# baumgach/PHiSeg-code

Hardware: AMD Instinct MI355X
Metric: training images/sec (ELBO step) phiseg_7_5 128x128 LIDC (higher is better)
Workload: dtype bf16; 1 GPU; phiseg_7_5 LIDC 128x128x1, 2 classes, bf16, batch norm, batch 64 per GPU, full ELBO training step (fwd + CE + KL + bwd + Adam); global_batch=64, parallelism=dp1

## Files before the change

### include/phx_debug.h

```cpp
#ifndef PHX_DEBUG_H
#define PHX_DEBUG_H
#ifdef __cplusplus
extern "C" {
#endif
int phx_debug_conv_policy(int large_maps, int big_tiles);
int phx_debug_pair_kernel_grid(int blocks);
int phx_debug_layer_norm_policy(int one_launch_max, int chunk);
#ifdef __cplusplus
}
#endif
#endif
```

### phiseg_code_amd/csrc/conv_c32.hip

```cpp
#include <stdlib.h>

#include <type_traits>

#include "phx_common.h"

namespace {

constexpr int C32_AI = 39;
constexpr int C32_NPL = 10;
constexpr int C32_STAGE = 40 * 1024;
constexpr int C32_PROW = 34 * 64;
constexpr int C32_LDS = 2 * C32_STAGE;

typedef __attribute__((address_space(3))) void* lds_ptr_t;

__device__ __forceinline__ unsigned lds_offset(const void* p) {
    return (unsigned)(uintptr_t)(const __attribute__((address_space(3))) unsigned char*)p;
}

__device__ unsigned long long* g_c32_trace = nullptr;
#define C32_TRACE(slot)                                                                          \
    do {                                                                                         \
        if (g_c32_trace && blockIdx.x == 0 && threadIdx.x == 0 && (slot) < 512)                   \
            g_c32_trace[slot] = __builtin_readcyclecounter();                                     \
    } while (0)

template <bool BIASACT, bool XF = false>
__global__ __launch_bounds__(256, 2) void k_conv3x3_c32(const unsigned short* __restrict__ x, const unsigned short* __restrict__ wpk,
                                                        unsigned short* __restrict__ y, const float* __restrict__ bias, int act,
                                                        float* __restrict__ stats_partial, int B, int H, int W, int tiles_x,
                                                        int tiles_y, int ntiles, const float* __restrict__ oscale, int stats_nrep, unsigned mgx, unsigned mgy,
                                                        const float* __restrict__ xscale = nullptr, const float* __restrict__ xshift = nullptr) {
    extern __shared__ __attribute__((aligned(16))) unsigned char smem[];
    const int wave = threadIdx.x >> 6, lane = threadIdx.x & 63;
    const int l31 = lane & 31, khalf = lane >> 5;

    bf16x8 fb[9][2];
#pragma unroll
    for (int tap = 0; tap < 9; ++tap)
#pragma unroll
        for (int ks = 0; ks < 2; ++ks)
            fb[tap][ks] = *reinterpret_cast<const bf16x8*>(wpk + ((tap * 32 + l31) * 32 + (ks * 2 + khalf) * 8));

    unsigned rel[C32_NPL], edge[C32_NPL];
#pragma unroll
    for (int n = 0; n < C32_NPL; ++n) {
        const int j = wave + 4 * n;
        const int e = j * 64 + lane, pp = e >> 2, slot = e & 3;
        const int py = pp / 34, px = pp - py * 34;
// ... 194 lines not shown
            const float s1 = s1v[0] + s1v[1], s2 = s2v[0] + s2v[1];
            const float a = s1 + __shfl_xor(s1, 32, 64);
            const float bq = s2 + __shfl_xor(s2, 32, 64);
            if (khalf == 0) {
                red[(wave * 2 + 0) * 32 + l31] = a;
                red[(wave * 2 + 1) * 32 + l31] = bq;
            }
            asm volatile("s_waitcnt lgkmcnt(0)\n\ts_barrier" ::: "memory");
            if (threadIdx.x < 64) {
                const int which = threadIdx.x >> 5, n = threadIdx.x & 31;
                float r0, r1, r2, r3;
                asm volatile("ds_read_b32 %0, %4\n\tds_read_b32 %1, %4 offset:256\n\tds_read_b32 %2, %4 offset:512\n\t"
                             "ds_read_b32 %3, %4 offset:768\n\ts_waitcnt lgkmcnt(0)"
                             : "=&v"(r0), "=&v"(r1), "=&v"(r2), "=&v"(r3)
                             : "v"(lds_offset(red + which * 32 + n))
                             : "memory");
                const float v = (r0 + r1) + (r2 + r3);
                if (stats_nrep > 0) atomicAdd(&stats_partial[((size_t)(t % stats_nrep) * 32 + n) * 2 + which], v);
                else stats_partial[((size_t)t * 2 + which) * 32 + n] = v;
            }
        }
    }
}

}

int phx_c32_set_trace(void* dev_buf) {
    PHX_CHECK_HIP(hipMemcpyToSymbol(HIP_SYMBOL(g_c32_trace), &dev_buf, sizeof(void*)));
    return PHX_OK;
}
bool phx_c32_enabled() { return true; }

int phx_c32_launch(const void* x, const void* wpk, void* y, const float* bias, int act, float* stats_partial, int B, int H, int W,
                   const float* oscale, int stats_nrep, void* stream, const float* xscale, const float* xshift) {
    const int tiles_x = W / 32, tiles_y = H / 16, ntiles = B * tiles_x * tiles_y;
    const int cap = 512;
    const int grid = ntiles < cap ? ntiles : cap;
    const bool ba = bias != nullptr || act != PHX_ACT_ID || oscale != nullptr;
    PHX_REQUIRE(ntiles < 65536, PHX_E_SHAPE, "conv3x3_c32: more than 65535 tiles");
    const unsigned mgx = (unsigned)((0x100000000ull + tiles_x - 1) / tiles_x), mgy = (unsigned)((0x100000000ull + tiles_y - 1) / tiles_y);
    if (xscale != nullptr) {
        PHX_REQUIRE(xshift != nullptr && !ba, PHX_E_INVAL, "conv3x3_c32: the input transform takes a plain epilogue");
        PHX_CHECK_HIP(hipFuncSetAttribute((const void*)k_conv3x3_c32<false, true>, hipFuncAttributeMaxDynamicSharedMemorySize, 160 * 1024));
        hipLaunchKernelGGL((k_conv3x3_c32<false, true>), dim3(grid), dim3(256), C32_LDS, (hipStream_t)stream, (const unsigned short*)x,
                           (const unsigned short*)wpk, (unsigned short*)y, bias, act, stats_partial, B, H, W, tiles_x, tiles_y, ntiles,
                           oscale, stats_nrep, mgx, mgy, xscale, xshift);
    } else if (ba) {
        PHX_CHECK_HIP(hipFuncSetAttribute((const void*)k_conv3x3_c32<true>, hipFuncAttributeMaxDynamicSharedMemorySize, 160 * 1024));
        hipLaunchKernelGGL((k_conv3x3_c32<true>), dim3(grid), dim3(256), C32_LDS, (hipStream_t)stream, (const unsigned short*)x,
                           (const unsigned short*)wpk, (unsigned short*)y, bias, act, stats_partial, B, H, W, tiles_x, tiles_y, ntiles,
                           oscale, stats_nrep, mgx, mgy, (const float*)nullptr, (const float*)nullptr);
    } else {
        PHX_CHECK_HIP(hipFuncSetAttribute((const void*)k_conv3x3_c32<false>, hipFuncAttributeMaxDynamicSharedMemorySize, 160 * 1024));
        hipLaunchKernelGGL((k_conv3x3_c32<false>), dim3(grid), dim3(256), C32_LDS, (hipStream_t)stream, (const unsigned short*)x,
                           (const unsigned short*)wpk, (unsigned short*)y, bias, act, stats_partial, B, H, W, tiles_x, tiles_y, ntiles,
                           oscale, stats_nrep, mgx, mgy, (const float*)nullptr, (const float*)nullptr);
    }
    PHX_CHECK_LAUNCH();
    return PHX_OK;
}
// ... 1 lines not shown
```

### phiseg_code_amd/csrc/conv_common.h

```cpp
#pragma once
#include <stdlib.h>

#include <type_traits>

#include "phx_common.h"
#include <cstring>

#ifndef PHX_ABLATE
#define PHX_ABLATE 0
#endif
#ifndef PHX_FRAG_DEPTH
#define PHX_FRAG_DEPTH 2
#endif
#define KC 32
#define ROWB 80
#define PITCH16 1536

struct MTile {
    int tws, ths, tb, tiles_x, tiles_y, tiles_b;
    unsigned mpw, mpp;
    int rpitch, ipitch;
};
static void mtile_magic(MTile* g) {
    const unsigned pw = (1u << g->tws) + 2, ph = (1u << g->ths) + 2;
    g->mpw = ((1u << 20) + pw - 1) / pw;
    g->mpp = ((1u << 20) + pw * ph - 1) / (pw * ph);
    g->rpitch = (int)pw * ROWB;
    g->ipitch = (int)ph * g->rpitch;
    if (g->tws == 3 && g->ths == 3) { g->rpitch = 56 * 16; g->ipitch = 560 * 16; }
    else if (g->tws == 2 && g->ths == 2) { g->rpitch = 36 * 16; g->ipitch = 224 * 16; }
    else if (g->tws == 1 && g->ths == 1) { g->rpitch = 22 * 16; g->ipitch = 92 * 16; }
}
__device__ __forceinline__ void patch_coords(const MTile& g, int pp, int pw, int ph, int* px, int* py, int* pb) {
    const int b = (int)(__umul24((unsigned)pp, g.mpp) >> 20);
    const int rem = pp - (int)__umul24((unsigned)b, (unsigned)(pw * ph));
// ... 59 lines not shown
```

### phiseg_code_amd/csrc/conv_mfma.hip

```cpp
#include "conv_common.h"

#ifdef PHX_DEBUG_BUILD
static int g_ws_policy = 1;
static int g_tile_policy = 1;
#else
static constexpr int g_ws_policy = 1, g_tile_policy = 1;
#endif

static bool fwd_big_tiles(int B, int H, int W, int K, int N) {
    if (!g_tile_policy || H % 32 != 0 || W % 16 != 0) return false;
    if (g_tile_policy == 2) return true;
    return (N % 128 == 0 || (N == 32 && K >= 128)) && (long)B * (H / 32) * (W / 16) >= 512;
}
static bool fwd_ws64(int B, int H, int W, int K, int N) {
    if (!g_ws_policy || H % 16 != 0 || W % 32 != 0 || N % 32 != 0 || K % 32 != 0) return false;
    if ((long)B * (H / 16) * (W / 32) >= 65536 || (double)B * H * W * (K > N ? K : N) >= 2147483648.0) return false;
    if (g_ws_policy >= 2) return true;
    if (N % 64 != 0 && K > 64) return false;
    return (long)B * (H / 16) * (W / 32) * (N / (N % 64 == 0 ? 64 : 32)) >= 512;
}
static MTile make_mtile_fwd(int B, int H, int W, int K, int N, bool allow_dma = true) {
    if (allow_dma && fwd_ws64(B, H, W, K, N)) {
        MTile g;
        g.tws = 5; g.ths = 4; g.tb = 1;
// ... 98 lines not shown
}
struct UnpadJob {
    const float* dw_pad; float* dw;
    int Cin, Cin_pad, Cout, ntap, blk0, reserved;
};
static_assert(sizeof(UnpadJob) == 40, "phx_unpad_filter_grad_multi: 40-byte job records (include/phx.h)");
__global__ void k_unpad_rows_acc_multi(const UnpadJob* __restrict__ jobs, int njobs) {
    int lo = 0, hi = njobs - 1;
    while (lo < hi) {
        const int mid = (lo + hi + 1) >> 1;
        if (jobs[mid].blk0 <= (int)blockIdx.x) lo = mid; else hi = mid - 1;
    }
    const UnpadJob j = jobs[lo];
    const int nblk = (lo + 1 < njobs ? jobs[lo + 1].blk0 : (int)gridDim.x) - j.blk0;
    if ((int)blockIdx.x < j.blk0 || nblk < 1) return;
    const int n = j.ntap * j.Cin * j.Cout;
    for (int i = (blockIdx.x - j.blk0) * blockDim.x + threadIdx.x; i < n; i += nblk * blockDim.x) {
        const int co = i % j.Cout, ci = (i / j.Cout) % j.Cin, t = j.ntap == 1 ? 4 : i / (j.Cout * j.Cin);
        j.dw[i] += j.dw_pad[((size_t)t * j.Cin_pad + ci) * j.Cout + co];
    }
}

int phx_c32_set_trace(void* dev_buf);
int phx_wgrad_set_debug(void* trace_buf, void* blocklog_buf, int which);
bool phx_c32_enabled();
int phx_c32_launch(const void* x, const void* wpk, void* y, const float* bias, int act, float* stats_partial, int B, int H, int W,
                   const float* oscale, int stats_nrep, void* stream, const float* xscale = nullptr, const float* xshift = nullptr);
struct Dual;
bool phx_pp_shape_ok(int B, int H, int W, int K, int N);
int phx_pp_set_trace(void* dev_buf);
int phx_pp_set_grid(int blocks);
int phx_pp_launch(const void* x, const void* wpk, void* y, const float* bias, int act, float* stats_partial, int B, int H, int W,
                  int K, int N, const float* oscale, int stats_nrep, Dual du, int dbg, void* stream);

struct EpiOpts {
    int stats_atomic;
    const float* oscale;
    float* y_f32;
    bool keep_slices;
};

struct XForm {
    const float *gamma, *beta;
    float eps;
    int G, act;
    unsigned short* a_out;
// ... 737 lines not shown
    return PHX_OK;
}

int phx_debug_set_trace(void* dev_buf) {
    if (int rc = phx_c32_set_trace(dev_buf)) return rc;
    if (int rc = phx_pp_set_trace(dev_buf)) return rc;
    if (int rc = phx_wgrad_set_debug(dev_buf, nullptr, 0)) return rc;
    unsigned long long* p = (unsigned long long*)dev_buf;
    PHX_CHECK_HIP(hipMemcpyToSymbol(HIP_SYMBOL(g_phx_trace), &p, sizeof(p)));
    return PHX_OK;
}

#ifdef PHX_DEBUG_BUILD
int phx_debug_conv_policy(int large_maps, int big_tiles) {
    PHX_REQUIRE(large_maps >= 0 && large_maps <= 2 && big_tiles >= 0 && big_tiles <= 2, PHX_E_INVAL, "debug_conv_policy: 0 never, 1 policy, 2 force");
    g_ws_policy = large_maps;
    g_tile_policy = big_tiles;
    return PHX_OK;
}

int phx_debug_pair_kernel_grid(int blocks) {
    PHX_REQUIRE(blocks >= 0, PHX_E_INVAL, "debug_pair_kernel_grid: blocks >= 0 (0: one per CU)");
    return phx_pp_set_grid(blocks);
}
#endif

int phx_debug_set_blocklog(void* dev_buf) {
    if (int rc = phx_wgrad_set_debug(nullptr, dev_buf, 1)) return rc;
    unsigned long long* p = (unsigned long long*)dev_buf;
    PHX_CHECK_HIP(hipMemcpyToSymbol(HIP_SYMBOL(g_phx_blocklog), &p, sizeof(p)));
    return PHX_OK;
}

static int q_tiles(int B, int H, int W, int K, int N) {
    MTile g = make_mtile_fwd(B, H, W, K, N);
    return g.tiles_x * g.tiles_y * g.tiles_b;
}

static int q_tiles_dual(int B, int H, int W, int K, int N) {
    MTile g = fwd_ws64(B, H, W, K, N) ? make_mtile_fwd(B, H, W, K, N) : make_mtile(B, H, W);
    return g.tiles_x * g.tiles_y * g.tiles_b;
}

static int fwd_ksplit(int B, int H, int W, int K, int N) {
    if (fwd_big_tiles(B, H, W, K, N)) return 1;
    MTile g = make_mtile(B, H, W);
// ... 285 lines not shown
```

### phiseg_code_amd/csrc/conv_wgrad.hip

```cpp
#include "conv_common.h"

template <int RB>
__device__ __forceinline__ int wswz(int pix, int byte_in_row) {
    if (RB == 128) return pix * 128 + (byte_in_row ^ (((pix >> 1) & 1) << 6));
    return pix * RB + byte_in_row;
}

template <int TCI, int TCO, bool BIGP, bool FAST16>
__device__ __forceinline__ void conv3x3_wgrad_body(const unsigned short* __restrict__ x0, const unsigned short* __restrict__ dy,
                                                   float* __restrict__ dw, float* __restrict__ ws, int B, int H, int W, int Cin,
                                                   int Cout, MTile g, int ntiles, int tiles_per_block, const int bx,
                                                   const int by, const int bz, const int gdx, const int gdy,
                                                   const unsigned short* __restrict__ x2 = nullptr, const int K1 = 0) {
    const bool src2 = x2 != nullptr && by * TCI >= K1;
    const unsigned short* __restrict__ x = src2 ? x2 : x0;
    const int xC = x2 == nullptr ? Cin : (src2 ? Cin - K1 : K1);
    const int xc0 = by * TCI - (src2 ? K1 : 0);
    constexpr int WI = TCI / 32, WJ = TCO / 32, WK = 4 / (WI * WJ);
    constexpr int RBX = TCI * 2, RBD = TCO * 2;
    constexpr int QX = TCI / 8, QD = TCO / 8;
    constexpr int NXI = ((BIGP ? 1024 : 400) * QX + 255) / 256;
    const int tw = 1 << g.tws, th = 1 << g.ths;
    const int pw = tw + 2, ph = th + 2;
    const int npatch = g.tb * ph * pw;
// ... 81 lines not shown
        if constexpr (PHX_ABLATE & 16) return;
        if constexpr (idx < NXI) {
            const int gx = ptx0 + (planx[idx] & 255) - 1, gy = pty0 + ((planx[idx] >> 8) & 255) - 1, gb = pb0 + (planx[idx] >> 16);
            const bool ok = planx[idx] >= 0 && gx >= 0 && gx < W && gy >= 0 && gy < H && gb < B;
            const unsigned vo = ok ? (unsigned)(((gb * H + gy) * W + gx) * xC * 2 + qxb) : 0xffffffffu;
            rx[idx] = __builtin_amdgcn_raw_buffer_load_b128(rsx, vo, xc0 * 2, 0);
        } else if constexpr (idx < NXI + QD) {
            constexpr int it = idx - NXI;
            const int ox = ptx0 + (pland[it] & 255), oy = pty0 + ((pland[it] >> 8) & 255), ob = pb0 + (pland[it] >> 16);
            const bool ok = ox < W && oy < H && ob < B;
            const unsigned vo = ok ? (unsigned)(((ob * H + oy) * W + ox) * Cout * 2 + qdb) : 0xffffffffu;
            rd[it] = __builtin_amdgcn_raw_buffer_load_b128(rsd, vo, co0 * 2, 0);
        }
    };
    auto prefetch_range = [&](auto self, auto lo, auto hi) {
        constexpr int l = decltype(lo)::value, h = decltype(hi)::value;
        if constexpr (l < h && l < NXI + QD) {
            prefetch_piece(lo);
            self(self, std::integral_constant<int, l + 1>(), hi);
        }
    };
    const int t_begin = bx * tiles_per_block;
    const int t_end = min(ntiles, t_begin + tiles_per_block);
    PHX_BLOCKLOG_BEGIN();
    PHX_TRACE(0);
    if (t_begin < t_end) {
        if constexpr (FAST16) {
            decode(t_begin);
            prefetch_range(prefetch_range, std::integral_constant<int, 0>(), std::integral_constant<int, NXI + QD>());
        } else {
            prefetch(t_begin);
        }
    }
    PHX_TRACE(1);

    for (int t = t_begin; t < t_end; ++t) {
        __syncthreads();
        if (t == t_begin) PHX_TRACE(2);
#pragma unroll
        for (int it = 0; it < NXI; ++it) {
            const int i = threadIdx.x + it * 256;
            if (planx[it] >= 0) *reinterpret_cast<u32x4*>(sX + wswz<RBX>(i / QX, (i % QX) * 16)) = rx[it];
        }
#pragma unroll
        for (int it = 0; it < QD; ++it) {
            const int i = threadIdx.x + it * 256;
            *reinterpret_cast<u32x4*>(sD + wswz<RBD>(i / QD, (i % QD) * 16)) = rd[it];
        }
        __syncthreads();
        if (t == t_begin) PHX_TRACE(3);
        const bool more = t + 1 < t_end;
        if constexpr (FAST16) { if (more) decode(t + 1); }
        else if (more) prefetch(t + 1);
        if (t == t_begin) PHX_TRACE(4);
        if (FAST16) {
            constexpr int NSTEP = 16 / WK;
            s16x4 fd[2][2], fx[2][9][2];
            auto read_step = [&](unsigned xb, unsigned db, auto parc, auto bufc) {
                constexpr int P = decltype(parc)::value;
                constexpr int Bf = decltype(bufc)::value;
                fd[Bf][0] = __builtin_amdgcn_ds_read_tr16_b64_v4i16((s16x4 __attribute__((address_space(3)))*)(smem + db + dcon[0]));
                fd[Bf][1] = __builtin_amdgcn_ds_read_tr16_b64_v4i16((s16x4 __attribute__((address_space(3)))*)(smem + db + dcon[1]));
#pragma unroll
                for (int kh = 0; kh < 3; ++kh)
#pragma unroll
                    for (int kw = 0; kw < 3; ++kw) {
                        const int par = (P + kh) & 1;
                        fx[Bf][kh * 3 + kw][0] = __builtin_amdgcn_ds_read_tr16_b64_v4i16(
                            (s16x4 __attribute__((address_space(3)))*)(smem + xb + kh * 18 * RBX + xcon[0][kw][par]));
                        fx[Bf][kh * 3 + kw][1] = __builtin_amdgcn_ds_read_tr16_b64_v4i16(
                            (s16x4 __attribute__((address_space(3)))*)(smem + xb + kh * 18 * RBX + xcon[1][kw][par]));
                    }
            };
            auto mfma_step = [&](auto bufc) {
                constexpr int Bf = decltype(bufc)::value;
                const s16x8 dtmp = {fd[Bf][0][0], fd[Bf][0][1], fd[Bf][0][2], fd[Bf][0][3], fd[Bf][1][0], fd[Bf][1][1], fd[Bf][1][2], fd[Bf][1][3]};
                const bf16x8 bfrag = __builtin_bit_cast(bf16x8, dtmp);
// ... 46 lines not shown
                }
                const s16x4 d0 = __builtin_amdgcn_ds_read_tr16_b64_v4i16(
                    (s16x4 __attribute__((address_space(3)))*)(sD + wswz<RBD>(mpix[0], chan_byte_d)));
                const s16x4 d1 = __builtin_amdgcn_ds_read_tr16_b64_v4i16(
                    (s16x4 __attribute__((address_space(3)))*)(sD + wswz<RBD>(mpix[1], chan_byte_d)));
                const s16x8 dtmp = {d0[0], d0[1], d0[2], d0[3], d1[0], d1[1], d1[2], d1[3]};
                const bf16x8 bfrag = __builtin_bit_cast(bf16x8, dtmp);
    #pragma unroll
                for (int kh = 0; kh < 3; ++kh)
    #pragma unroll
                    for (int kw = 0; kw < 3; ++kw) {
                        const int sh = kh * pw + kw;
                        const s16x4 a0 = __builtin_amdgcn_ds_read_tr16_b64_v4i16(
                            (s16x4 __attribute__((address_space(3)))*)(sX + wswz<RBX>(ppix[0] + sh, chan_byte_x)));
                        const s16x4 a1 = __builtin_amdgcn_ds_read_tr16_b64_v4i16(
                            (s16x4 __attribute__((address_space(3)))*)(sX + wswz<RBX>(ppix[1] + sh, chan_byte_x)));
                        const s16x8 atmp = {a0[0], a0[1], a0[2], a0[3], a1[0], a1[1], a1[2], a1[3]};
                        const bf16x8 afrag = __builtin_bit_cast(bf16x8, atmp);
                        acc[kh * 3 + kw] = __builtin_amdgcn_mfma_f32_32x32x16_bf16(afrag, bfrag, acc[kh * 3 + kw], 0, 0, 0);
                    }
            }
        }
    }
    PHX_TRACE(5);
    if (ws) {
        const size_t cb = (size_t)bz * gdy + by;
        float* wp = ws + ((cb * gdx + bx) * WK + wk) * (size_t)(9 * TCI * TCO);
#pragma unroll
        for (int k = 0; k < 9; ++k)
#pragma unroll
            for (int r = 0; r < 16; ++r) {
                const int cil = wi * 32 + (r & 3) + 8 * (r >> 2) + 4 * (lane >> 5);
                wp[(k * TCI + cil) * TCO + wj * 32 + (lane & 31)] = acc[k][r];
            }
    } else {
        const int co = co0 + wj * 32 + (lane & 31);
#pragma unroll
        for (int k = 0; k < 9; ++k)
#pragma unroll
            for (int r = 0; r < 16; ++r) {
                const int ci = ci0 + wi * 32 + (r & 3) + 8 * (r >> 2) + 4 * (lane >> 5);
                atomicAdd(&dw[((size_t)k * Cin + ci) * Cout + co], acc[k][r]);
            }
    }
    PHX_TRACE(6);
    PHX_BLOCKLOG_END();
}

template <int TCI, int TCO, bool BIGP, bool FAST16>
__global__ __launch_bounds__(256, 1) void k_conv3x3_wgrad(const unsigned short* __restrict__ x,
                                                          const unsigned short* __restrict__ dy,
                                                          float* __restrict__ dw, float* __restrict__ ws, int B, int H,
                                                          int W, int Cin, int Cout, MTile g, int ntiles,
                                                          int tiles_per_block, const unsigned short* __restrict__ x2, int K1) {
    conv3x3_wgrad_body<TCI, TCO, BIGP, FAST16>(x, dy, dw, ws, B, H, W, Cin, Cout, g, ntiles, tiles_per_block, blockIdx.x,
                                               blockIdx.y, blockIdx.z, gridDim.x, gridDim.y, x2, K1);
}
struct WgMJob {
    const unsigned short* x; const unsigned short* dy; float* dw; float* ws;
    int B, H, W, Cin, Cout;
    MTile g;
    int ntiles, tpb, gdx, gdy, gdz, blk0;
    const unsigned short* x2; int K1, pad_;
};
template <int TCI, int TCO, bool BIGP>
__global__ __launch_bounds__(256, 1) void k_conv3x3_wgrad_multi(const WgMJob* __restrict__ jobs, int njobs) {
    int lo = 0, hi = njobs - 1;
    while (lo < hi) {
        const int mid = (lo + hi + 1) >> 1;
// ... 55 lines not shown
        const int pp = e / QX, ps = e % QX;
        const int p = RBX == 128 ? (ps ^ (((pp >> 1) & 1) << 2)) : ps;
        return pp < NPATCH ? ((pp % 18) | ((pp / 18) << 8) | (p << 16)) : -1;
    };
    auto plan_d = [&](int n) -> int {
        const int e = (wave + 4 * n) * 64 + lane;
        const int m = e / QD, ps = e % QD;
        const int p = RBD == 128 ? (ps ^ (((m >> 1) & 1) << 2)) : ps;
        return (m & 15) | ((m >> 4) << 8) | (p << 16);
    };
    int planx[RPLAN ? XN : 1], pland[RPLAN ? DN : 1];
    if constexpr (RPLAN) {
#pragma unroll
        for (int n = 0; n < XN; ++n) planx[n] = plan_x(n);
#pragma unroll
        for (int n = 0; n < DN; ++n) pland[n] = plan_d(n);
    }
    const __amdgpu_buffer_rsrc_t rsx = __builtin_amdgcn_make_buffer_rsrc((void*)x, 0, (int)((unsigned)B * H * W * xC * 2u), 0x00020000);
    const __amdgpu_buffer_rsrc_t rsd = __builtin_amdgcn_make_buffer_rsrc((void*)dy, 0, (int)((unsigned)B * H * W * Cout * 2u), 0x00020000);
    typedef __attribute__((address_space(3))) void* lds_ptr_t;

    const int t_begin = bx * tiles_per_block;
    const int t_end = min(ntiles, t_begin + tiles_per_block);
    PHX_BLOCKLOG_BEGIN();
    for (int t = t_begin; t < t_end; ++t) {
        int tt = t;
        const int tx0 = (tt % g.tiles_x) << 4; tt /= g.tiles_x;
        const int ty0 = (tt % g.tiles_y) << 4; tt /= g.tiles_y;
        const int b0 = tt;
        __syncthreads();
#pragma unroll
        for (int n = 0; n < XN; ++n) {
            if (wave + 4 * n < XI) {
                int pk;
                if constexpr (RPLAN) pk = planx[n]; else pk = plan_x(n);
                const int gx = tx0 + (pk & 255) - 1, gy = ty0 + ((pk >> 8) & 255) - 1;
                const bool ok = pk >= 0 && gx >= 0 && gx < W && gy >= 0 && gy < H;
                const unsigned vo = ok ? (unsigned)((((b0 * H + gy) * W + gx) * xC) * 2 + (pk >> 16) * 16) : 0xffffffffu;
                __builtin_amdgcn_raw_ptr_buffer_load_lds(rsx, (lds_ptr_t)(smem + (wave + 4 * n) * 1024), 16, vo, xc0 * 2, 0, 0);
            }
        }
#pragma unroll
        for (int n = 0; n < DN; ++n) {
            int pk;
            if constexpr (RPLAN) pk = pland[n]; else pk = plan_d(n);
            const int ox = tx0 + (pk & 255), oy = ty0 + ((pk >> 8) & 255);
            const bool ok = ox < W && oy < H;
// ... 94 lines not shown
                        p[(k * 4 + q) * 64] = f32x4_t{acc[k][4 * q], acc[k][4 * q + 1], acc[k][4 * q + 2], acc[k][4 * q + 3]};
            __syncthreads();
            if (sel == 0)
#pragma unroll
                for (int k = 0; k < 9; ++k)
#pragma unroll
                    for (int q = 0; q < 4; ++q) {
                        const f32x4_t v = p[(k * 4 + q) * 64];
                        acc[k][4 * q] += v[0]; acc[k][4 * q + 1] += v[1]; acc[k][4 * q + 2] += v[2]; acc[k][4 * q + 3] += v[3];
                    }
        }
    }
    if (WK == 1 || wk == 0) {
        const size_t cb = (size_t)bz * gdy + by;
        float* wp = ws + (cb * gdx + bx) * (size_t)(9 * TCI * TCO);
#pragma unroll
        for (int k = 0; k < 9; ++k)
#pragma unroll
            for (int r = 0; r < 16; ++r) {
                const int cil = wi * 32 + (r & 3) + 8 * (r >> 2) + 4 * (lane >> 5);
                wp[(k * TCI + cil) * TCO + wj * 32 + (lane & 31)] = acc[k][r];
            }
    }
    PHX_BLOCKLOG_END();
}

template <int TCI, int TCO>
__global__ __launch_bounds__(256, 2) void k_conv3x3_wgrad_dma(const unsigned short* __restrict__ x,
                                                              const unsigned short* __restrict__ dy, float* __restrict__ ws,
                                                              int B, int H, int W, int Cin, int Cout, MTile g, int ntiles,
                                                              int tiles_per_block, const unsigned short* __restrict__ x2, int K1,
                                                              const float* __restrict__ xscale, const float* __restrict__ xshift) {
    conv3x3_wgrad_dma_body<TCI, TCO>(x, dy, ws, B, H, W, Cin, Cout, g, ntiles, tiles_per_block, blockIdx.x, blockIdx.y, blockIdx.z,
                                     gridDim.x, gridDim.y, x2, K1, xscale, xshift);
}
template <int TCI, int TCO>
__global__ __launch_bounds__(256, 2) void k_conv3x3_wgrad_dma_multi(const WgMJob* __restrict__ jobs, int njobs) {
    int lo = 0, hi = njobs - 1;
    while (lo < hi) {
        const int mid = (lo + hi + 1) >> 1;
        if (jobs[mid].blk0 <= (int)blockIdx.x) lo = mid; else hi = mid - 1;
    }
    const WgMJob j = jobs[lo];
    const int local = blockIdx.x - j.blk0;
    conv3x3_wgrad_dma_body<TCI, TCO>(j.x, j.dy, j.ws, j.B, j.H, j.W, j.Cin, j.Cout, j.g, j.ntiles, j.tpb, local % j.gdx,
                                     (local / j.gdx) % j.gdy, local / (j.gdx * j.gdy), j.gdx, j.gdy, j.x2, j.K1);
}
// ... 109 lines not shown
                auto slot = [&](auto kc) {
                    constexpr int k = decltype(kc)::value, kh = k / 3, kw = k % 3, Rs = (SI + kh) & 3;
                    const s16x8 atmp = {fx[Rs][kw][0][0], fx[Rs][kw][0][1], fx[Rs][kw][0][2], fx[Rs][kw][0][3],
                                        fx[Rs][kw][1][0], fx[Rs][kw][1][1], fx[Rs][kw][1][2], fx[Rs][kw][1][3]};
                    acc[k] = __builtin_amdgcn_mfma_f32_32x32x16_bf16(__builtin_bit_cast(bf16x8, atmp), bfrag, acc[k], 0, 0, 0);
                    if constexpr (more) {
                        if constexpr (k < 2) rd_d(IC(SI + 1), kc);
                        else if constexpr (k < 8) rd_x(IC(SI + 3), IC((k - 2) >> 1), IC((k - 2) & 1));
                    }
                    __builtin_amdgcn_sched_barrier(0);
                };
                slot(IC(0)); slot(IC(1)); slot(IC(2)); slot(IC(3)); slot(IC(4)); slot(IC(5)); slot(IC(6)); slot(IC(7)); slot(IC(8));
                self(self, IC(SI + 1));
            }
        };
        steps(steps, IC(0));
#undef IC
    };
#define WPP_BARRIER() asm volatile("s_waitcnt vmcnt(0) lgkmcnt(0)\n\ts_barrier" ::: "memory")
    const int t_begin = bx * tiles_per_block;
    const int t_end = min(ntiles, t_begin + tiles_per_block);
    const int n = t_end - t_begin;
    const int nA = (n + 1) >> 1, nh = half ? (n >> 1) : nA;
    PHX_BLOCKLOG_BEGIN();
    if (half == 0 && nh > 0) load_tile(t_begin);
    WPP_BARRIER();
    if (half) {
        if (nh > 0) load_tile(t_begin + 1);
        WPP_BARRIER();
    }
    for (int k = 0; k < nA; ++k) {
        if (k < nh) compute();
        WPP_BARRIER();
        if (k + 1 < nh) load_tile(t_begin + half + 2 * (k + 1));
        WPP_BARRIER();
    }
    if (half == 0) WPP_BARRIER();
    typedef __attribute__((ext_vector_type(4))) float f32x4_t;
    f32x4_t* const pr = reinterpret_cast<f32x4_t*>(smem) + (size_t)lw * (9 * 4 * 64) + lane;
    if (half)
#pragma unroll
        for (int k = 0; k < 9; ++k)
#pragma unroll
            for (int q = 0; q < 4; ++q) pr[(k * 4 + q) * 64] = f32x4_t{acc[k][4 * q], acc[k][4 * q + 1], acc[k][4 * q + 2], acc[k][4 * q + 3]};
    WPP_BARRIER();
#undef WPP_BARRIER
    if (half == 0) {
        const size_t cb = (size_t)bz * gdy + by;
        float* wp = ws + (cb * gdx + bx) * (size_t)(9 * TCI * TCO);
#pragma unroll
        for (int k = 0; k < 9; ++k) {
#pragma unroll
            for (int q = 0; q < 4; ++q) {
                const f32x4_t v = pr[(k * 4 + q) * 64];
                acc[k][4 * q] += v[0]; acc[k][4 * q + 1] += v[1]; acc[k][4 * q + 2] += v[2]; acc[k][4 * q + 3] += v[3];
            }
#pragma unroll
            for (int r = 0; r < 16; ++r) {
                const int cil = wi * 32 + (r & 3) + 8 * (r >> 2) + 4 * (lane >> 5);
                wp[(k * TCI + cil) * TCO + wj * 32 + (lane & 31)] = acc[k][r];
            }
        }
    }
    PHX_BLOCKLOG_END();
}

__global__ __launch_bounds__(512, 1) void k_conv3x3_wgrad_pp(const unsigned short* __restrict__ x, const unsigned short* __restrict__ dy,
                                                             float* __restrict__ ws, int B, int H, int W, int Cin, int Cout, MTile g,
                                                             int ntiles, int tiles_per_block, const unsigned short* __restrict__ x2,
                                                             int K1) {
    conv3x3_wgrad_pp_body(x, dy, ws, B, H, W, Cin, Cout, g, ntiles, tiles_per_block, blockIdx.x, blockIdx.y, blockIdx.z, gridDim.x,
                          gridDim.y, x2, K1);
}
__global__ __launch_bounds__(512, 1) void k_conv3x3_wgrad_pp_multi(const WgMJob* __restrict__ jobs, int njobs) {
    int lo = 0, hi = njobs - 1;
    while (lo < hi) {
        const int mid = (lo + hi + 1) >> 1;
        if (jobs[mid].blk0 <= (int)blockIdx.x) lo = mid; else hi = mid - 1;
    }
    const WgMJob j = jobs[lo];
    const int local = blockIdx.x - j.blk0;
    const int cb = j.gdy * j.gdz, t = local >> 3;
    const int c = t % cb, bx = (t / cb) * 8 + (local & 7);
    if (bx >= j.gdx) return;
    conv3x3_wgrad_pp_body(j.x, j.dy, j.ws, j.B, j.H, j.W, j.Cin, j.Cout, j.g, j.ntiles, j.tpb, bx, c % j.gdy, c / j.gdy, j.gdx, j.gdy,
                          j.x2, j.K1);
}
// ... 328 lines not shown
```

Baseline: 6732 images/s.

## Pipeline c32 conv patch DMA across tiles and overlap it with stores

```diff
diff --git a/include/phx_debug.h b/include/phx_debug.h
--- a/include/phx_debug.h
+++ b/include/phx_debug.h
@@ -5,6 +5,7 @@
 #endif
 int phx_debug_conv_policy(int large_maps, int big_tiles);
 int phx_debug_pair_kernel_grid(int blocks);
+int phx_debug_c32_kernel_grid(int blocks, int stats_nrep);
 int phx_debug_layer_norm_policy(int one_launch_max, int chunk);
 #ifdef __cplusplus
 }
diff --git a/phiseg_code_amd/csrc/conv_c32.hip b/phiseg_code_amd/csrc/conv_c32.hip
--- a/phiseg_code_amd/csrc/conv_c32.hip
+++ b/phiseg_code_amd/csrc/conv_c32.hip
@@ -2,7 +2,7 @@
 
 #include <type_traits>
 
-#include "phx_common.h"
+#include "conv_common.h"
 
 namespace {
 
@@ -19,12 +19,20 @@
 }
 
 __device__ unsigned long long* g_c32_trace = nullptr;
+#if PHX_C32_PIPELINE
+#define C32_TRACE(slot)                                                                          \
+    do {                                                                                         \
+        if ((slot) < 512) PHX_TRACE_TO(trc, slot, __builtin_readcyclecounter());                  \
+    } while (0)
+#else
 #define C32_TRACE(slot)                                                                          \
     do {                                                                                         \
         if (g_c32_trace && blockIdx.x == 0 && threadIdx.x == 0 && (slot) < 512)                   \
             g_c32_trace[slot] = __builtin_readcyclecounter();                                     \
     } while (0)
-
+#endif
+
+#if !PHX_C32_PIPELINE
 template <bool BIASACT, bool XF = false>
 __global__ __launch_bounds__(256, 2) void k_conv3x3_c32(const unsigned short* __restrict__ x, const unsigned short* __restrict__ wpk,
                                                         unsigned short* __restrict__ y, const float* __restrict__ bias, int act,
@@ -265,6 +273,295 @@
         }
     }
 }
+#else
+constexpr int C32_RED = 32 * 1024;
+constexpr int C32_XFC = C32_AI * 1024;
+
+template <bool BIASACT, bool XF = false>
+__global__ __launch_bounds__(256, 2) void k_conv3x3_c32(const unsigned short* __restrict__ x, const unsigned short* __restrict__ wpk,
+                                                        unsigned short* __restrict__ y, const float* __restrict__ bias, int act,
+                                                        float* __restrict__ stats_partial, int B, int H, int W, int tiles_x,
+                                                        int tiles_y, int ntiles, const float* __restrict__ oscale, int stats_nrep, unsigned mgx, unsigned mgy,
+                                                        const float* __restrict__ xscale = nullptr, const float* __restrict__ xshift = nullptr) {
+    extern __shared__ __attribute__((aligned(16))) unsigned char smem[];
+    const unsigned long long trv = (unsigned long long)g_c32_trace;
+    const int wave = threadIdx.x >> 6, lane = threadIdx.x & 63;
+    const int l31 = lane & 31, khalf = lane >> 5;
+
+    unsigned rel[C32_NPL], edge[C32_NPL];
+#pragma unroll
+    for (int n = 0; n < C32_NPL; ++n) {
+        const int j = wave + 4 * n;
+        const int e = j * 64 + lane, pp = e >> 2, slot = e & 3;
+        const int py = pp / 34, px = pp - py * 34;
+        rel[n] = (unsigned)((py * W + px) * 64 + ((slot ^ ((px >> 2) & 3)) << 4));
+        edge[n] = (j < C32_AI && pp < 612) ? (unsigned)((px == 0) | ((px == 33) << 1) | ((py == 0) << 2) | ((py == 17) << 3)) : 15u;
+    }
+    const __amdgpu_buffer_rsrc_t rsx = __builtin_amdgcn_make_buffer_rsrc((void*)x, 0, (int)((unsigned)B * H * W * 64u), 0x00020000);
+    auto decode = [&](int t, int* tx0, int* ty0, int* b0) {
+        const int q1 = tiles_x == 1 ? t : (int)__umulhi((unsigned)t, mgx);
+        *tx0 = (t - q1 * tiles_x) << 5;
+        const int q2 = tiles_y == 1 ? q1 : (int)__umulhi((unsigned)q1, mgy);
+        *ty0 = (q1 - q2 * tiles_y) << 4;
+        *b0 = q2;
+    };
+    unsigned pbase = 0, pout = 0, pnone = 0;
+    int pstage = 0;
+    auto patch_setup = [&](int t, int stage) {
+        int tx0, ty0, b0;
+        decode(t, &tx0, &ty0, &b0);
+        pbase = (unsigned)(((b0 * H + ty0 - 1) * W + tx0 - 1) * 64);
+        pout = (tx0 == 0 ? 1u : 0u) | (tx0 + 32 >= W ? 2u : 0u) | (ty0 == 0 ? 4u : 0u) | (ty0 + 16 >= H ? 8u : 0u);
+        pstage = stage;
+    };
+    auto issue_piece = [&](auto nc) {
+        constexpr int n = decltype(nc)::value;
+        const int j = wave + 4 * n;
+        if (j < C32_AI) {
+            const bool bad = edge[n] == 15u || (edge[n] & pout) != 0u;
+            const unsigned vo = (bad ? 0xffffffffu : pbase + rel[n]) | pnone;
+            __builtin_amdgcn_raw_ptr_buffer_load_lds(rsx, (lds_ptr_t)(smem + pstage * C32_STAGE + j * 1024), 16, (int)vo, 0, 0, 0);
+        }
+    };
+    auto issue_range = [&](auto self, auto lo, auto hi) {
+        constexpr int l = decltype(lo)::value, h = decltype(hi)::value;
+        if constexpr (l < h && l < C32_NPL) {
+            issue_piece(lo);
+            self(self, std::integral_constant<int, l + 1>(), hi);
+        }
+    };
+    const int gstep = (int)gridDim.x;
+    int slot = blockIdx.x, t = phx_band8(slot, ntiles);
+    patch_setup(t, 0);
+    issue_range(issue_range, std::integral_constant<int, 0>(), std::integral_constant<int, C32_NPL>());
+
+    bf16x8 fb[9][2];
+#pragma unroll
+    for (int tap = 0; tap < 9; ++tap)
+#pragma unroll
+        for (int ks = 0; ks < 2; ++ks)
+            fb[tap][ks] = *reinterpret_cast<const bf16x8*>(wpk + ((tap * 32 + l31) * 32 + (ks * 2 + khalf) * 8));
+    {
+        const bool two = slot + gstep < ntiles;
+        patch_setup(phx_band8(two ? slot + gstep : slot, ntiles), 1);
+        pnone = two ? 0u : 0xffffffffu;
+        issue_range(issue_range, std::integral_constant<int, 0>(), std::integral_constant<int, C32_NPL>());
+        pnone = 0u;
+    }
+    float bv = 0.f, sv = 1.f, xcf = 0.f;
+    if constexpr (BIASACT) {
+        const __amdgpu_buffer_rsrc_t rsb = __builtin_amdgcn_make_buffer_rsrc((void*)bias, 0, bias ? 128 : 0, 0x00020000);
+        const __amdgpu_buffer_rsrc_t rss = __builtin_amdgcn_make_buffer_rsrc((void*)oscale, 0, oscale ? 128 : 0, 0x00020000);
+        bv = __uint_as_float(__builtin_amdgcn_raw_buffer_load_b32(rsb, l31 * 4, 0, 0));
+        sv = __uint_as_float(__builtin_amdgcn_raw_buffer_load_b32(rss, l31 * 4, 0, 0));
+    }
+    if constexpr (XF) xcf = ((threadIdx.x & 32) ? xshift : xscale)[threadIdx.x & 31];
+
+    unsigned aK[3][2];
+#pragma unroll
+    for (int kw = 0; kw < 3; ++kw)
+#pragma unroll
+        for (int ks = 0; ks < 2; ++ks)
+            aK[kw][ks] = (unsigned)((wave * 4 * 34 + l31 + kw) * 64 + (((ks * 2 + khalf) ^ (((l31 + kw) >> 2) & 3)) << 4));
+    const int odd = lane & 1;
+    unsigned long long* const trc = blockIdx.x == 0 ? phx_uniform_ptr(trv) : nullptr;
+    if constexpr (BIASACT) {
+        if (oscale == nullptr) sv = 1.f;
+        asm volatile("" : "+v"(bv), "+v"(sv));
+    }
+    if constexpr (XF) {
+        if (threadIdx.x < 64) *reinterpret_cast<float*>(smem + C32_XFC + threadIdx.x * 4) = xcf;
+    }
+
+    for (int it = 0; slot < ntiles; slot += gstep, t = phx_band8(slot, ntiles), ++it) {
+        const int cur = it & 1;
+        const unsigned char* st = smem + cur * C32_STAGE;
+        const bool more1 = slot + gstep < ntiles, more2 = slot + 2 * gstep < ntiles;
+        C32_TRACE(it * 8 + 0);
+        if (it == 0) asm volatile("s_waitcnt vmcnt(0) lgkmcnt(0)\n\ts_barrier" ::: "memory");
+        else if (more1) asm volatile("s_waitcnt vmcnt(17)\n\ts_barrier" ::: "memory");
+        else asm volatile("s_waitcnt vmcnt(8)\n\ts_barrier" ::: "memory");
+        C32_TRACE(it * 8 + 1);
+        if constexpr (XF) {
+            int tx0c, ty0c, b0c;
+            decode(t, &tx0c, &ty0c, &b0c);
+            const bool e_l = tx0c == 0, e_r = tx0c + 32 >= W, e_t = ty0c == 0, e_b = ty0c + 16 >= H;
+            int tid = threadIdx.x;
+            asm volatile("" : "+v"(tid));
+            const int sp = tid & 3;
+            typedef __attribute__((ext_vector_type(4))) unsigned u32x4_t;
+            typedef __attribute__((ext_vector_type(4))) float f32x4_t;
+            f32x4_t c0, c1, d0, d1;
+            u32x4_t r[10];
+            unsigned qa[10];
+#pragma unroll
+            for (int n = 0; n < 10; ++n) {
+                const int pp = (tid >> 2) + 64 * n;
+                const int py = (int)(((unsigned)pp * 1928u) >> 16), px = pp - py * 34;
+                qa[n] = lds_offset(st + pp * 64 + ((sp ^ ((px >> 2) & 3)) << 4));
+            }
+            asm volatile("ds_read_b128 %0, %14\n\tds_read_b128 %1, %14 offset:16\n\tds_read_b128 %2, %14 offset:128\n\t"
+                         "ds_read_b128 %3, %14 offset:144\n\tds_read_b128 %4, %15\n\tds_read_b128 %5, %16\n\tds_read_b128 %6, %17\n\t"
+                         "ds_read_b128 %7, %18\n\tds_read_b128 %8, %19\n\tds_read_b128 %9, %20\n\tds_read_b128 %10, %21\n\t"
+                         "ds_read_b128 %11, %22\n\tds_read_b128 %12, %23\n\tds_read_b128 %13, %24\n\ts_waitcnt lgkmcnt(0)"
+                         : "=&v"(c0), "=&v"(c1), "=&v"(d0), "=&v"(d1), "=&v"(r[0]), "=&v"(r[1]), "=&v"(r[2]), "=&v"(r[3]), "=&v"(r[4]),
+                           "=&v"(r[5]), "=&v"(r[6]), "=&v"(r[7]), "=&v"(r[8]), "=&v"(r[9])
+                         : "v"(lds_offset(smem + C32_XFC + sp * 32)), "v"(qa[0]), "v"(qa[1]), "v"(qa[2]), "v"(qa[3]), "v"(qa[4]), "v"(qa[5]),
+                           "v"(qa[6]), "v"(qa[7]), "v"(qa[8]), "v"(qa[9])
+                         : "memory");
+            const float xsc[8] = {c0[0], c0[1], c0[2], c0[3], c1[0], c1[1], c1[2], c1[3]};
+            const float xsh[8] = {d0[0], d0[1], d0[2], d0[3], d1[0], d1[1], d1[2], d1[3]};
+#pragma unroll
+            for (int n = 0; n < 10; ++n) {
+                const int pp = (tid >> 2) + 64 * n;
+                const int py = (int)(((unsigned)pp * 1928u) >> 16), px = pp - py * 34;
+                const bool outside = (px == 0 && e_l) || (px == 33 && e_r) || (py == 0 && e_t) || (py == 17 && e_b);
+                u32x4_t o;
+#pragma unroll
+                for (int k = 0; k < 4; ++k) {
+                    const float a0 = fmaxf(fmaf(__uint_as_float(r[n][k] << 16), xsc[2 * k], xsh[2 * k]), 0.f);
+                    const float a1 = fmaxf(fmaf(__uint_as_float(r[n][k] & 0xffff0000u), xsc[2 * k + 1], xsh[2 * k + 1]), 0.f);
+                    o[k] = outside ? 0u : f2bf_pk(a0, a1);
+                }
+                if (pp < 612) asm volatile("ds_write_b128 %0, %1" : : "v"(qa[n]), "v"(o) : "memory");
+            }
+            asm volatile("s_waitcnt lgkmcnt(0)\n\ts_barrier" ::: "memory");
+        }
+        C32_TRACE(it * 8 + 2);
+
+        f32x16 acc[4];
+#pragma unroll
+        for (int i = 0; i < 4; ++i)
+#pragma unroll
+            for (int r = 0; r < 16; ++r) acc[i][r] = 0.f;
+        bf16x8 fa[2][6];
+        auto read_a = [&](auto gc) {
+            constexpr int g = decltype(gc)::value;
+            constexpr int ks = g / 3, kw = g % 3;
+#pragma unroll
+            for (int rr = 0; rr < 6; ++rr)
+                fa[g & 1][rr] = *reinterpret_cast<const bf16x8*>(st + aK[kw][ks] + rr * C32_PROW);
+        };
+        read_a(std::integral_constant<int, 0>());
+        auto groups = [&](auto self, auto gc) {
+            constexpr int g = decltype(gc)::value;
+            if constexpr (g < 6) {
+                constexpr int ks = g / 3, kw = g % 3;
+                if constexpr (g + 1 < 6) read_a(std::integral_constant<int, g + 1>());
+                __builtin_amdgcn_sched_barrier(0);
+#pragma unroll
+                for (int kh = 0; kh < 3; ++kh)
+#pragma unroll
+                    for (int i = 0; i < 4; ++i)
+                        acc[i] = __builtin_amdgcn_mfma_f32_32x32x16_bf16(fa[g & 1][i + kh], fb[kh * 3 + kw][ks], acc[i], 0, 0, 0);
+                __builtin_amdgcn_sched_barrier(0);
+                self(self, std::integral_constant<int, g + 1>());
+            }
+        };
+        groups(groups, std::integral_constant<int, 0>());
+        C32_TRACE(it * 8 + 3);
+        asm volatile("s_waitcnt lgkmcnt(0)\n\ts_barrier" ::: "memory");
+        C32_TRACE(it * 8 + 4);
+
+        if constexpr (BIASACT) {
+#pragma unroll
+            for (int i = 0; i < 4; ++i)
+#pragma unroll
+                for (int r = 0; r < 16; ++r) acc[i][r] = fmaf(acc[i][r], sv, bv);
+            if (act == PHX_ACT_RELU) {
+#pragma unroll
+                for (int i = 0; i < 4; ++i)
+#pragma unroll
+                    for (int r = 0; r < 16; ++r) acc[i][r] = fmaxf(acc[i][r], 0.f);
+            } else if (act != PHX_ACT_ID) {
+#pragma unroll
+                for (int i = 0; i < 4; ++i)
+#pragma unroll
+                    for (int r = 0; r < 16; ++r) acc[i][r] = act_fwd(acc[i][r], act);
+            }
+        }
+        typedef __attribute__((ext_vector_type(2))) float f32x2_t;
+        f32x2_t s1v = {0.f, 0.f}, s2v = {0.f, 0.f};
+        const unsigned psel = odd ? 0x03020706u : 0x05040100u;
+        unsigned char* lwp = smem + cur * C32_STAGE + (wave * 128 + 4 * khalf + odd) * 64 + (l31 & ~1) * 2;
+        auto pack = [&](auto stc) {
+#pragma unroll
+            for (int i = 0; i < 4; ++i)
+#pragma unroll
+                for (int rp = 0; rp < 8; ++rp) {
+                    const int r0 = 2 * rp;
+                    float v0 = acc[i][r0], v1 = acc[i][r0 + 1];
+                    const unsigned w2 = f2bf_pk(v0, v1);
+                    if constexpr (decltype(stc)::value) {
+                        const f32x2_t rv = {__uint_as_float(w2 << 16), __uint_as_float(w2 & 0xffff0000u)};
+                        s1v += rv;
+                        s2v += rv * rv;
+                        __builtin_amdgcn_sched_barrier(0);
+                    }
+                    const unsigned nb = (unsigned)__builtin_amdgcn_mov_dpp((int)w2, 0xB1, 0xf, 0xf, true);
+                    *reinterpret_cast<unsigned*>(lwp + (i * 32 + (r0 & 3) + 8 * (r0 >> 2)) * 64) = __builtin_amdgcn_perm(nb, w2, psel);
+                }
+        };
+        if (stats_partial) pack(std::true_type()); else pack(std::false_type());
+        float* const red = reinterpret_cast<float*>(smem + cur * C32_STAGE + C32_RED);
+        if (stats_partial) {
+            const float s1 = s1v[0] + s1v[1], s2 = s2v[0] + s2v[1];
+            const float a = s1 + __shfl_xor(s1, 32, 64);
+            const float bq = s2 + __shfl_xor(s2, 32, 64);
+            if (khalf == 0) {
+                red[(wave * 2 + 0) * 32 + l31] = a;
+                red[(wave * 2 + 1) * 32 + l31] = bq;
+            }
+        }
+        C32_TRACE(it * 8 + 5);
+        asm volatile("s_waitcnt lgkmcnt(0)\n\ts_barrier" ::: "memory");
+        int tx0, ty0, b0;
+        decode(t, &tx0, &ty0, &b0);
+        const int mt = threadIdx.x >> 2, q = threadIdx.x & 3;
+        const unsigned char* lr = smem + cur * C32_STAGE + mt * 64 + q * 16;
+        unsigned short* yp = y + (((size_t)b0 * H + ty0 + (mt >> 5)) * W + tx0 + (mt & 31)) * 32 + q * 8;
+        const size_t ystep = (size_t)2 * W * 32;
+        const unsigned la = lds_offset(lr);
+        uint4 v[8];
+        asm volatile("ds_read_b128 %0, %8\n\tds_read_b128 %1, %8 offset:4096\n\tds_read_b128 %2, %8 offset:8192\n\t"
+                     "ds_read_b128 %3, %8 offset:12288\n\tds_read_b128 %4, %8 offset:16384\n\tds_read_b128 %5, %8 offset:20480\n\t"
+                     "ds_read_b128 %6, %8 offset:24576\n\tds_read_b128 %7, %8 offset:28672\n\ts_waitcnt lgkmcnt(0)"
+                     : "=&v"(v[0]), "=&v"(v[1]), "=&v"(v[2]), "=&v"(v[3]), "=&v"(v[4]), "=&v"(v[5]), "=&v"(v[6]), "=&v"(v[7])
+                     : "v"(la)
+                     : "memory");
+        float sred = 0.f;
+        const bool reducer = stats_partial != nullptr && threadIdx.x < 64;
+        if (reducer) {
+            float r0, r1, r2, r3;
+            asm volatile("ds_read_b32 %0, %4\n\tds_read_b32 %1, %4 offset:256\n\tds_read_b32 %2, %4 offset:512\n\t"
+                         "ds_read_b32 %3, %4 offset:768\n\ts_waitcnt lgkmcnt(0)"
+                         : "=&v"(r0), "=&v"(r1), "=&v"(r2), "=&v"(r3)
+                         : "v"(lds_offset(red + threadIdx.x))
+                         : "memory");
+            sred = (r0 + r1) + (r2 + r3);
+        }
+        asm volatile("s_barrier" ::: "memory");
+        if (more2) {
+            patch_setup(phx_band8(slot + 2 * gstep, ntiles), cur);
+#define C32_DMA_STORE(k) issue_piece(std::integral_constant<int, k>()); *reinterpret_cast<uint4*>(yp + k * ystep) = v[k]
+            C32_DMA_STORE(0); C32_DMA_STORE(1); C32_DMA_STORE(2); C32_DMA_STORE(3);
+            C32_DMA_STORE(4); C32_DMA_STORE(5); C32_DMA_STORE(6); C32_DMA_STORE(7);
+#undef C32_DMA_STORE
+            issue_piece(std::integral_constant<int, 8>());
+            issue_piece(std::integral_constant<int, 9>());
+        } else {
+#pragma unroll
+            for (int k = 0; k < 8; ++k) *reinterpret_cast<uint4*>(yp + k * ystep) = v[k];
+        }
+        C32_TRACE(it * 8 + 6);
+        if (reducer) {
+            const int which = threadIdx.x >> 5, n = threadIdx.x & 31;
+            if (stats_nrep > 0) atomicAdd(&stats_partial[((size_t)(t % stats_nrep) * 32 + n) * 2 + which], sred);
+            else stats_partial[((size_t)t * 2 + which) * 32 + n] = sred;
+        }
+    }
+}
+#endif
 
 }
 
@@ -274,11 +571,23 @@
 }
 bool phx_c32_enabled() { return true; }
 
+#ifdef PHX_DEBUG_BUILD
+static int g_c32_grid = 0, g_c32_nrep = 0;
+int phx_c32_set_grid(int blocks, int stats_nrep) {
+    g_c32_grid = blocks;
+    g_c32_nrep = stats_nrep;
+    return PHX_OK;
+}
+#else
+static constexpr int g_c32_grid = 0, g_c32_nrep = 0;
+#endif
+
 int phx_c32_launch(const void* x, const void* wpk, void* y, const float* bias, int act, float* stats_partial, int B, int H, int W,
                    const float* oscale, int stats_nrep, void* stream, const float* xscale, const float* xshift) {
     const int tiles_x = W / 32, tiles_y = H / 16, ntiles = B * tiles_x * tiles_y;
-    const int cap = 512;
+    const int cap = g_c32_grid > 0 ? g_c32_grid : 512;
     const int grid = ntiles < cap ? ntiles : cap;
+    if (g_c32_nrep > 0 && stats_partial != nullptr) stats_nrep = g_c32_nrep;
     const bool ba = bias != nullptr || act != PHX_ACT_ID || oscale != nullptr;
     PHX_REQUIRE(ntiles < 65536, PHX_E_SHAPE, "conv3x3_c32: more than 65535 tiles");
     const unsigned mgx = (unsigned)((0x100000000ull + tiles_x - 1) / tiles_x), mgy = (unsigned)((0x100000000ull + tiles_y - 1) / tiles_y);
diff --git a/phiseg_code_amd/csrc/conv_common.h b/phiseg_code_amd/csrc/conv_common.h
--- a/phiseg_code_amd/csrc/conv_common.h
+++ b/phiseg_code_amd/csrc/conv_common.h
@@ -11,6 +11,9 @@
 #endif
 #ifndef PHX_FRAG_DEPTH
 #define PHX_FRAG_DEPTH 2
+#endif
+#ifndef PHX_C32_PIPELINE
+#define PHX_C32_PIPELINE 1
 #endif
 #define KC 32
 #define ROWB 80
diff --git a/phiseg_code_amd/csrc/conv_mfma.hip b/phiseg_code_amd/csrc/conv_mfma.hip
--- a/phiseg_code_amd/csrc/conv_mfma.hip
+++ b/phiseg_code_amd/csrc/conv_mfma.hip
@@ -144,6 +144,7 @@
 }
 
 int phx_c32_set_trace(void* dev_buf);
+int phx_c32_set_grid(int blocks, int stats_nrep);
 int phx_wgrad_set_debug(void* trace_buf, void* blocklog_buf, int which);
 bool phx_c32_enabled();
 int phx_c32_launch(const void* x, const void* wpk, void* y, const float* bias, int act, float* stats_partial, int B, int H, int W,
@@ -927,6 +928,11 @@
 int phx_debug_pair_kernel_grid(int blocks) {
     PHX_REQUIRE(blocks >= 0, PHX_E_INVAL, "debug_pair_kernel_grid: blocks >= 0 (0: one per CU)");
     return phx_pp_set_grid(blocks);
+}
+
+int phx_debug_c32_kernel_grid(int blocks, int stats_nrep) {
+    PHX_REQUIRE(blocks >= 0 && stats_nrep >= 0, PHX_E_INVAL, "debug_c32_kernel_grid: blocks >= 0 (0: 512), stats_nrep >= 0 (0: per-tile rows)");
+    return phx_c32_set_grid(blocks, stats_nrep);
 }
 #endif
 
diff --git a/phiseg_code_amd/csrc/conv_wgrad.hip b/phiseg_code_amd/csrc/conv_wgrad.hip
--- a/phiseg_code_amd/csrc/conv_wgrad.hip
+++ b/phiseg_code_amd/csrc/conv_wgrad.hip
@@ -1,4 +1,28 @@
 #include "conv_common.h"
+
+#if PHX_C32_PIPELINE
+#define WG_DEBUG_BEGIN()                                                                                               \
+    const unsigned long long blv = (unsigned long long)g_phx_blocklog;                                                 \
+    const unsigned long long bl_t0 = __builtin_readcyclecounter()
+#define WG_DEBUG_END()                                         \
+    do {                                                       \
+        unsigned long long* const blg = phx_uniform_ptr(blv);  \
+        PHX_BLOCKLOG_END_TO(blg);                              \
+    } while (0)
+#define WG_TRACE_BEGIN() const unsigned long long trv = (unsigned long long)g_phx_trace
+#define WG_TRACE_ISSUED()                                                                                                \
+    const unsigned long long t_issued = __builtin_readcyclecounter();                                                    \
+    unsigned long long* const trc = (blockIdx.x | blockIdx.y | blockIdx.z) == 0 ? phx_uniform_ptr(trv) : nullptr;        \
+    PHX_TRACE_TO(trc, 0, bl_t0);                                                                                         \
+    PHX_TRACE_TO(trc, 1, t_issued)
+#define WG_TRACE(slot) PHX_TRACE_TO(trc, slot, __builtin_readcyclecounter())
+#else
+#define WG_DEBUG_BEGIN() PHX_BLOCKLOG_BEGIN()
+#define WG_DEBUG_END() PHX_BLOCKLOG_END()
+#define WG_TRACE_BEGIN() PHX_TRACE(0)
+#define WG_TRACE_ISSUED() PHX_TRACE(1)
+#define WG_TRACE(slot) PHX_TRACE(slot)
+#endif
 
 template <int RB>
 __device__ __forceinline__ int wswz(int pix, int byte_in_row) {
@@ -127,8 +151,8 @@
     };
     const int t_begin = bx * tiles_per_block;
     const int t_end = min(ntiles, t_begin + tiles_per_block);
-    PHX_BLOCKLOG_BEGIN();
-    PHX_TRACE(0);
+    WG_DEBUG_BEGIN();
+    WG_TRACE_BEGIN();
     if (t_begin < t_end) {
         if constexpr (FAST16) {
             decode(t_begin);
@@ -137,11 +161,11 @@
             prefetch(t_begin);
         }
     }
-    PHX_TRACE(1);
+    WG_TRACE_ISSUED();
 
     for (int t = t_begin; t < t_end; ++t) {
         __syncthreads();
-        if (t == t_begin) PHX_TRACE(2);
+        if (t == t_begin) WG_TRACE(2);
 #pragma unroll
         for (int it = 0; it < NXI; ++it) {
             const int i = threadIdx.x + it * 256;
@@ -153,11 +177,11 @@
             *reinterpret_cast<u32x4*>(sD + wswz<RBD>(i / QD, (i % QD) * 16)) = rd[it];
         }
         __syncthreads();
-        if (t == t_begin) PHX_TRACE(3);
+        if (t == t_begin) WG_TRACE(3);
         const bool more = t + 1 < t_end;
         if constexpr (FAST16) { if (more) decode(t + 1); }
         else if (more) prefetch(t + 1);
-        if (t == t_begin) PHX_TRACE(4);
+        if (t == t_begin) WG_TRACE(4);
         if (FAST16) {
             constexpr int NSTEP = 16 / WK;
             s16x4 fd[2][2], fx[2][9][2];
@@ -250,7 +274,7 @@
             }
         }
     }
-    PHX_TRACE(5);
+    WG_TRACE(5);
     if (ws) {
         const size_t cb = (size_t)bz * gdy + by;
         float* wp = ws + ((cb * gdx + bx) * WK + wk) * (size_t)(9 * TCI * TCO);
@@ -271,8 +295,8 @@
                 atomicAdd(&dw[((size_t)k * Cin + ci) * Cout + co], acc[k][r]);
             }
     }
-    PHX_TRACE(6);
-    PHX_BLOCKLOG_END();
+    WG_TRACE(6);
+    WG_DEBUG_END();
 }
 
 template <int TCI, int TCO, bool BIGP, bool FAST16>
@@ -374,7 +398,7 @@
 
     const int t_begin = bx * tiles_per_block;
     const int t_end = min(ntiles, t_begin + tiles_per_block);
-    PHX_BLOCKLOG_BEGIN();
+    WG_DEBUG_BEGIN();
     for (int t = t_begin; t < t_end; ++t) {
         int tt = t;
         const int tx0 = (tt % g.tiles_x) << 4; tt /= g.tiles_x;
@@ -515,7 +539,7 @@
                 wp[(k * TCI + cil) * TCO + wj * 32 + (lane & 31)] = acc[k][r];
             }
     }
-    PHX_BLOCKLOG_END();
+    WG_DEBUG_END();
 }
 
 template <int TCI, int TCO>
@@ -671,7 +695,7 @@
     const int t_end = min(ntiles, t_begin + tiles_per_block);
     const int n = t_end - t_begin;
     const int nA = (n + 1) >> 1, nh = half ? (n >> 1) : nA;
-    PHX_BLOCKLOG_BEGIN();
+    WG_DEBUG_BEGIN();
     if (half == 0 && nh > 0) load_tile(t_begin);
     WPP_BARRIER();
     if (half) {
@@ -711,7 +735,7 @@
             }
         }
     }
-    PHX_BLOCKLOG_END();
+    WG_DEBUG_END();
 }
 
 __global__ __launch_bounds__(512, 1) void k_conv3x3_wgrad_pp(const unsigned short* __restrict__ x, const unsigned short* __restrict__ dy,
```

Result: no change. 6731 images/s (-0.0%).
